# javieryu/nn_distributed_training

Hardware: NVIDIA H100
Metric: consensus node-rounds/sec (DiNNO, dist_mnist_PAPER; rounds/sec x graph nodes) (higher is better)
Workload: dtype fp64

## Files before the change

### nn_distributed_training_b200/ops/csrc/mnist_cl64.cu

```cuda
#include "mnist_device.cuh"

namespace nndt {
namespace mnist {

namespace cl64 {

constexpr int NT = 512, CL = 4, CELLS = 36, KC = 108, WS = 116, HS = 68;
constexpr int PXR = 10 * HW;
constexpr int KT = (KC + 7) / 8;
constexpr int HR = 68;
NNDT_DEVINL int hr(int j) { return (j >> 4) * 17 + (j & 15); }
constexpr int PART_WC = 0, PART_BC = 75, PART_B1 = 78, PART_W2 = 142, PART_B2 = 782, PART_LOSS = 792, PART_N = 793;

template <int MS>
struct Smem {
  static constexpr int NO = MS / CL;
  static constexpr bool kDoublePix = MS <= 32;
  static constexpr int PXS = kDoublePix ? PXR + 2 : PXR;
  double w[HID * WS];
  double a[MS * WS];
  double h[MS * HS];
  alignas(16) unsigned char img[kDoublePix ? MS * PXS * 8 : MS * PXS];
  double lut[kDoublePix ? 1 : 256];
  double h_loc[NO * HR > CL * 80 ? NO * HR : CL * 80];
  double dh_loc[NO * HID];
  double part[800];
  double w2[NCLS * HR];
  alignas(16) double b1[HID];
  alignas(16) double b2[16];
  double wc[80];
  double dz[NO * 16];
  double red[NO];
  int sidx[MS];
  int label[MS];
  float valid[MS];
  unsigned char arg[MS * KC];
};
static_assert(sizeof(Smem<16>) <= 227 * 1024 && sizeof(Smem<32>) <= 227 * 1024 && sizeof(Smem<64>) <= 227 * 1024,
              "shared memory budget");

NNDT_DEVINL double wmax(double v) {
#pragma unroll
  for (int o = 16; o > 0; o >>= 1) v = fmax(v, __shfl_xor_sync(0xffffffffu, v, o));
  return v;
}
template <int H>
NNDT_DEVINL void fold_half(double (&v)[16], int lane) {
  const bool up = (lane & (2 * H)) != 0;
#pragma unroll
  for (int i = 0; i < H; ++i) {
    const double send = up ? v[i] : v[i + H], keep = up ? v[i + H] : v[i];
    v[i] = keep + __shfl_xor_sync(0xffffffffu, send, 2 * H);
  }
}
NNDT_DEVINL void warp_reduce_scatter16(double (&v)[16], int lane) {
  fold_half<8>(v, lane); fold_half<4>(v, lane); fold_half<2>(v, lane); fold_half<1>(v, lane);
  v[0] += __shfl_xor_sync(0xffffffffu, v[0], 1);
}
NNDT_DEVINL void stamp(long long* prof, int idx, int tid) {
  if (prof != nullptr && tid == 0) {
    long long t;
    asm volatile("mov.u64 %0, %%globaltimer;" : "=l"(t));
    prof[idx] = t;
  }
}

template <int MS>
__global__ void __cluster_dims__(CL, 1, 1) __launch_bounds__(NT, 1)
mnist_cl64_train_kernel(const Args a, const GenericShape gs) {
  using SM = Smem<MS>;
  constexpr int NO = SM::NO, PXS = SM::PXS;
  constexpr bool kDoublePix = SM::kDoublePix;
  static_assert(MS % 16 == 0 && NO <= NT / 32, "tile geometry");
  static_assert(CELLS % 2 == 0 && NCLS % 2 == 0 && 32 + NCLS / 2 <= NT, "16-byte parameter copies");
  extern __shared__ __align__(16) unsigned char smem_raw[];
  SM& sm = *reinterpret_cast<SM*>(smem_raw);
  const int tid = threadIdx.x, warp = tid >> 5, lane = tid & 31;
  const int l = blockIdx.z, bsplit = blockIdx.y, nsplit = gridDim.y;
  const int c = (int)cluster_rank();
  const double* th = reinterpret_cast<const double*>(a.theta) + (size_t)l * a.n_pad;
  const double pmean = gs.mean, pis = gs.inv_std;
  const bool u8 = a.x_is_u8 != 0;
  double* imgd = reinterpret_cast<double*>(sm.img);
  auto pix = [&](int s, int p) -> double {
    if constexpr (kDoublePix) return imgd[s * PXS + p];
    else if (u8) return sm.lut[sm.img[s * PXR + p]];
    else return (double)__ldg(reinterpret_cast<const float*>(a.x) + (size_t)sm.sidx[s] * 784 + 6 * HW * c + p);
  };
  long long* prof = a.prof != nullptr ? a.prof + ((l * nsplit + bsplit) * CL + c) * 64 : nullptr;
  stamp(prof, 0, tid);

  const int call = a.calls != nullptr ? a.calls[l] : 0;
  const BatchGeom bg = batch_geom<true>(a, l, call);
  if (tid < MS) {
    int idx = 0, lab = 0; float ok = 0.f;
    const uint32_t t = (uint32_t)(bsplit * MS + tid);
    if (t < bg.bs) {
      ok = 1.f;
      idx = a.direct ? (int)(l * a.batch + t) : bg.shard_off + (int)feistel_permute(bg.start + t, bg.m, bg.key);
      lab = (int)a.y[idx];
    }
    sm.sidx[tid] = idx; sm.valid[tid] = ok; sm.label[tid] = lab;
  }
  if constexpr (!kDoublePix)
    if (tid < 256) sm.lut[tid] = ((double)tid * (1.0 / 255.0) - pmean) * pis;
  __syncthreads();
  constexpr int NU8 = (MS * 35 + NT - 1) / NT, NF4 = kDoublePix ? (MS * 70 + NT - 1) / NT : 1;
  uint2 pu[NU8]; float4 pf[NF4];
  if (u8) {
#pragma unroll
    for (int i = 0; i < NU8; ++i) {
      const int o = tid + i * NT;
      pu[i] = make_uint2(0, 0);
      if (o < MS * 35) {
        const int s = o / 35, q = o - s * 35;
        if (sm.valid[s] != 0.f)
          pu[i] = *reinterpret_cast<const uint2*>(reinterpret_cast<const unsigned char*>(a.x) + (size_t)sm.sidx[s] * 784 + 6 * HW * c + 8 * q);
      }
    }
  } else if constexpr (kDoublePix) {
#pragma unroll
    for (int i = 0; i < NF4; ++i) {
      const int o = tid + i * NT;
      pf[i] = make_float4(0.f, 0.f, 0.f, 0.f);
      if (o < MS * 70) {
        const int s = o / 70, q = o - s * 70;
        if (sm.valid[s] != 0.f)
          pf[i] = *reinterpret_cast<const float4*>(reinterpret_cast<const float*>(a.x) + (size_t)sm.sidx[s] * 784 + 6 * HW * c + 4 * q);
      }
    }
  }
  if (u8) {
#pragma unroll
    for (int i = 0; i < NU8; ++i) {
      const int o = tid + i * NT;
      if (o < MS * 35) {
        const int s = o / 35, q = o - s * 35;
        if constexpr (kDoublePix) {
          const uint32_t w[2] = {pu[i].x, pu[i].y};
          double* dst = imgd + s * PXS + 8 * q;
#pragma unroll
          for (int j = 0; j < 8; ++j) dst[j] = ((double)((w[j >> 2] >> (8 * (j & 3))) & 0xff) * (1.0 / 255.0) - pmean) * pis;
        } else {
          *reinterpret_cast<uint2*>(sm.img + s * PXR + 8 * q) = pu[i];
        }
      }
    }
  } else if constexpr (kDoublePix) {
#pragma unroll
    for (int i = 0; i < NF4; ++i) {
      const int o = tid + i * NT;
      if (o < MS * 70) {
        double* dst = imgd + (o / 70) * PXS + 4 * (o % 70);
        dst[0] = pf[i].x; dst[1] = pf[i].y; dst[2] = pf[i].z; dst[3] = pf[i].w;
      }
    }
  }
  stamp(prof, 1, tid);
  pdl_wait();
  pdl_launch_dependents();
  stamp(prof, 2, tid);

  constexpr int NW2 = (NCLS * HID + NT - 1) / NT;
  double wcv = 0.0, w2v[NW2];
  if (tid < 75) wcv = __ldcg(th + a.off_wc + tid);
  else if (tid < 78) wcv = __ldcg(th + a.off_bc + (tid - 75));
#pragma unroll
  for (int i = 0; i < NW2; ++i) {
    const int o = tid + i * NT;
    w2v[i] = o < NCLS * HID ? __ldcg(th + a.off_w2 + o) : 0.0;
  }
  for (int o = tid; o < HID * KC / 2; o += NT) {
    const int j = o / (KC / 2), r = o - j * (KC / 2), ch = r / (CELLS / 2), q = 2 * (r - ch * (CELLS / 2));
    cp_async16(sm.w + j * WS + ch * CELLS + q, th + a.off_w1 + (size_t)j * FC1_IN + ch * NPOOL + CELLS * c + q);
  }
  if (tid < HID / 2) cp_async16(sm.b1 + 2 * tid, th + a.off_b1 + 2 * tid);
  else if (tid >= 32 && tid < 32 + NCLS / 2) cp_async16(sm.b2 + 2 * (tid - 32), th + a.off_b2 + 2 * (tid - 32));
  cp_async_commit();
  if (tid < 78) sm.wc[tid] = wcv;
#pragma unroll
  for (int i = 0; i < NW2; ++i) {
    const int o = tid + i * NT;
    if (o < NCLS * HID) sm.w2[(o / HID) * HR + hr(o % HID)] = w2v[i];
  }
  __syncthreads();
  stamp(prof, 3, tid);

  for (int it = tid; it < MS * CELLS; it += NT) {
    const int s = it / CELLS, cell = it - s * CELLS;
    const int pr = cell / PHW, px = cell - pr * PHW;
    const int p0 = (2 * pr) * HW + 2 * px;
    double patch[6][6];
    if constexpr (kDoublePix) {
      const double* src = imgd + s * PXS + p0;
#pragma unroll
      for (int r = 0; r < 6; ++r)
#pragma unroll
        for (int q = 0; q < 6; q += 2) {
          const double2 v = *reinterpret_cast<const double2*>(src + r * HW + q);
          patch[r][q] = v.x; patch[r][q + 1] = v.y;
        }
    } else {
#pragma unroll
      for (int r = 0; r < 6; ++r)
#pragma unroll
        for (int q = 0; q < 6; ++q) patch[r][q] = pix(s, p0 + r * HW + q);
    }
    const bool ok = sm.valid[s] != 0.f;
#pragma unroll 1
    for (int ch = 0; ch < F; ++ch) {
      double a00 = 0, a01 = 0, a10 = 0, a11 = 0;
#pragma unroll
      for (int ky = 0; ky < KS; ++ky)
#pragma unroll
        for (int kx = 0; kx < KS; ++kx) {
          const double w = sm.wc[ch * 25 + ky * 5 + kx];
          a00 += w * patch[ky][kx]; a01 += w * patch[ky][kx + 1];
          a10 += w * patch[ky + 1][kx]; a11 += w * patch[ky + 1][kx + 1];
        }
      double m = a00; int ai = 0;
      if (a01 > m) { m = a01; ai = 1; }
      if (a10 > m) { m = a10; ai = 2; }
      if (a11 > m) { m = a11; ai = 3; }
      m += sm.wc[75 + ch];
      m = (ok && m > 0.0) ? m : 0.0;
      sm.a[s * WS + ch * CELLS + cell] = m;
      sm.arg[s * KC + ch * CELLS + cell] = (unsigned char)(ai | (m > 0.0 ? 4 : 0));
    }
  }
  cp_async_wait<0>();
  __syncthreads();
  stamp(prof, 4, tid);

  {
    constexpr int NJ1 = MS == 64 ? 2 : 1, NGRP = 8 / NJ1;
    if (warp < (MS / 16) * NGRP) {
      const int m0 = 16 * (warp / NGRP), n0 = 8 * NJ1 * (warp % NGRP);
      double acc[NJ1][4];
      zero(acc);
      gemm<NJ1>(acc, m0, n0, KC, lane, at(sm.a, WS), at_t(sm.w, WS));
#pragma unroll
      for (int j = 0; j < NJ1; ++j)
#pragma unroll
        for (int i = 0; i < 4; ++i) sm.h[frow(m0, lane, i) * HS + fcol(n0 + 8 * j, lane, i)] = acc[j][i];
    }
  }
  stamp(prof, 5, tid);
  cluster_sync();
  stamp(prof, 6, tid);
  if (c == 0 && tid == 0 && a.calls != nullptr) {
    if (a.arrive == nullptr || nsplit == 1) a.calls[l] = call + 1;
    else if (atomicAdd(a.arrive + l, 1u) == (unsigned)nsplit - 1) { a.arrive[l] = 0; a.calls[l] = call + 1; }
  }

  const int s0 = c * NO;
  const double inv_bs = 1.0 / (double)(bg.bs ? bg.bs : 1);
  if (warp < NO) {
    const int sl = warp, s = s0 + sl;
    double hv[2];
#pragma unroll
    for (int q = 0; q < 2; ++q) {
      const int j = lane + 32 * q;
      const double* src = sm.h + s * HS + j;
      double v = sm.b1[j];
#pragma unroll
      for (int r = 0; r < CL; ++r) v += ld_dsmem(map_to(src, (uint32_t)r));
      hv[q] = v > 0.0 ? v : 0.0;
      sm.h_loc[sl * HR + hr(j)] = hv[q];
    }
    __syncwarp();
    double zp[2];
#pragma unroll
    for (int r = 0; r < 2; ++r) {
      const int o = lane + 32 * r, cc = o >> 2, part = o & 3;
      double v = 0.0;
      if (o < 4 * NCLS) {
#pragma unroll
        for (int jj = 0; jj < 16; ++jj) v += sm.h_loc[sl * HR + part * 17 + jj] * sm.w2[cc * HR + part * 17 + jj];
      }
      v += __shfl_xor_sync(0xffffffffu, v, 1);
      v += __shfl_xor_sync(0xffffffffu, v, 2);
      zp[r] = v;
    }
    static_assert(NCLS > 8 && NCLS <= 16, "two rounds of four lanes per class");
    const double z0 = __shfl_sync(0xffffffffu, zp[0], (4 * lane) & 31), z1 = __shfl_sync(0xffffffffu, zp[1], (4 * lane) & 31);
    const bool cls = lane < NCLS;
    const double zc = cls ? (lane < 8 ? z0 : z1) + sm.b2[lane] : -1.0e300;
    const double mx = wmax(zc);
    const double se = warp_sum(cls ? exp(zc - mx) : 0.0);
    const double lse = mx + log(se);
    const int y = sm.label[s];
    const double ok = (double)sm.valid[s];
    const double dzc = cls ? ok * inv_bs * (exp(zc - lse) - (lane == y ? 1.0 : 0.0)) : 0.0;
    if (cls) sm.dz[sl * 16 + lane] = dzc;
    if (lane == y) sm.red[sl] = ok * (lse - zc);
    double dh[2] = {0.0, 0.0};
#pragma unroll
    for (int cc = 0; cc < NCLS; ++cc) {
      const double d = __shfl_sync(0xffffffffu, dzc, cc);
      dh[0] += d * sm.w2[cc * HR + hr(lane)];
      dh[1] += d * sm.w2[cc * HR + hr(lane + 32)];
    }
#pragma unroll
    for (int q = 0; q < 2; ++q) sm.dh_loc[sl * HID + lane + 32 * q] = hv[q] > 0.0 ? dh[q] : 0.0;
  }
  __syncthreads();
  for (int o = tid; o < NCLS * HID; o += NT) {
    const int cc = o >> 6, j = o & 63;
    double v = 0.0;
    for (int sl = 0; sl < NO; ++sl) v += sm.dz[sl * 16 + cc] * sm.h_loc[sl * HR + hr(j)];
    sm.part[PART_W2 + o] = v;
  }
  if (tid < HID) {
    double v = 0.0;
    for (int sl = 0; sl < NO; ++sl) v += sm.dh_loc[sl * HID + tid];
    sm.part[PART_B1 + tid] = v;
  } else if (tid >= 64 && tid < 64 + NCLS) {
    double v = 0.0;
    for (int sl = 0; sl < NO; ++sl) v += sm.dz[sl * 16 + (tid - 64)];
    sm.part[PART_B2 + (tid - 64)] = v;
  } else if (tid == 96) {
    double v = 0.0;
    for (int sl = 0; sl < NO; ++sl) v += sm.red[sl];
    sm.part[PART_LOSS] = v * inv_bs;
  }
  stamp(prof, 7, tid);
  cluster_sync();
  stamp(prof, 8, tid);
  double* gp = reinterpret_cast<double*>(a.grad_part) + ((size_t)l * nsplit + bsplit) * a.n_pad;
  {
    constexpr int NE = PART_N - PART_B1, PER = (NE + CL - 1) / CL;
    const int o = PART_B1 + c * PER + tid;
    if (tid < PER && o < PART_N) {
      double v = 0.0;
#pragma unroll
      for (int r = 0; r < CL; ++r) v += ld_dsmem(map_to(sm.part + o, (uint32_t)r));
      if (o < PART_W2) gp[a.off_b1 + (o - PART_B1)] = v;
      else if (o < PART_B2) gp[a.off_w2 + (o - PART_W2)] = v;
      else if (o < PART_LOSS) gp[a.off_b2 + (o - PART_B2)] = v;
      else {
        a.loss_part[l * nsplit + bsplit] = (float)v;
        if (a.loss_mirror != nullptr) a.loss_mirror[l * nsplit + bsplit] = (float)v;
      }
    }
  }
  for (int o = tid; o < MS * HID; o += NT) {
    const int s = o >> 6, j = o & 63, r = s / NO;
    sm.h[s * HS + j] = ld_dsmem(map_to(sm.dh_loc + (s - r * NO) * HID + j, (uint32_t)r));
  }
  __syncthreads();
  stamp(prof, 9, tid);

  constexpr int NP2 = (MS / 16) * (KT / 2), NR2 = (NP2 + NT / 32 - 1) / (NT / 32);
  static_assert(KT % 2 == 0 && KC * MS + (NT / 32) * 16 <= HID * WS, "da1 and the conv-grad warp sums fit in the W slice");
  double acc2[NR2][2][4];
#pragma unroll
  for (int r = 0; r < NR2; ++r) {
    zero(acc2[r]);
    const int p = warp + r * (NT / 32);
    if (p < NP2) gemm<2>(acc2[r], 16 * (p / (KT / 2)), 16 * (p % (KT / 2)), HID, lane, at(sm.h, HS), at(sm.w, WS));
  }
  __syncthreads();
  stamp(prof, 10, tid);
  double* da1 = sm.w;
#pragma unroll
  for (int r = 0; r < NR2; ++r) {
    const int p = warp + r * (NT / 32);
    if (p < NP2) {
      const int m0 = 16 * (p / (KT / 2)), n0 = 16 * (p % (KT / 2));
#pragma unroll
      for (int jt = 0; jt < 2; ++jt)
#pragma unroll
        for (int i = 0; i < 4; ++i) {
          const int s = frow(m0, lane, i), k = fcol(n0 + 8 * jt, lane, i);
          if (k < KC) da1[k * MS + s] = (sm.arg[s * KC + k] & 4) ? acc2[r][jt][i] : 0.0;
        }
    }
  }
  __syncthreads();
  stamp(prof, 11, tid);
  {
    constexpr int NP3 = (HID / 16) * (KT / 2);
#pragma unroll 1
    for (int p = warp; p < NP3; p += NT / 32) {
      const int m0 = 16 * (p / (KT / 2)), n0 = 16 * (p % (KT / 2));
      double acc[2][4];
      zero(acc);
      gemm<2>(acc, m0, n0, MS, lane, at_t(sm.h, HS), at(sm.a, WS));
#pragma unroll
      for (int jt = 0; jt < 2; ++jt)
#pragma unroll
        for (int i = 0; i < 4; i += 2) {
          const int j = frow(m0, lane, i), k = fcol(n0 + 8 * jt, lane, i);
          if (k < KC) {
            const int ch = k / CELLS, cell = k - ch * CELLS;
            *reinterpret_cast<double2*>(gp + a.off_w1 + (size_t)j * FC1_IN + ch * NPOOL + CELLS * c + cell) =
                make_double2(acc[jt][i], acc[jt][i + 1]);
          }
        }
    }
  }
  constexpr int KW = 3, NRUN = MS * 3;
  static_assert(KS * KW < NT / 32 && F * KS <= 16, "conv-grad work split");
  double* wsums = sm.w + KC * MS;
  auto pix2 = [&](int s, int p) -> double2 {
    if constexpr (kDoublePix) return *reinterpret_cast<const double2*>(imgd + s * PXS + p);
    else return make_double2(pix(s, p), pix(s, p + 1));
  };
  if (warp < KS * KW) {
    const int ky = warp / KW;
    double acc[16];
#pragma unroll
    for (int i = 0; i < 16; ++i) acc[i] = 0.0;
#pragma unroll 1
    for (int r = tid - ky * KW * 32; r < NRUN; r += KW * 32) {
      const int s = r % MS, pr = r / MS;
      const int rb = (2 * pr + ky) * HW;
      double x0[6], x1[6];
#pragma unroll
      for (int px = 0; px < PHW; ++px) {
        const int p = rb + 2 * px;
        if (px == 0) {
#pragma unroll
          for (int q = 0; q < 6; q += 2) {
            const double2 u = pix2(s, p + q), v = pix2(s, p + HW + q);
            x0[q] = u.x; x0[q + 1] = u.y; x1[q] = v.x; x1[q + 1] = v.y;
          }
        } else {
#pragma unroll
          for (int q = 0; q < 4; ++q) { x0[q] = x0[q + 2]; x1[q] = x1[q + 2]; }
          const double2 u = pix2(s, p + 4), v = pix2(s, p + HW + 4);
          x0[4] = u.x; x0[5] = u.y; x1[4] = v.x; x1[5] = v.y;
        }
#pragma unroll
        for (int ch = 0; ch < F; ++ch) {
          const int k = ch * CELLS + pr * PHW + px;
          const double g = da1[k * MS + s];
          const int ai = sm.arg[s * KC + k] & 3;
          const double g00 = ai == 0 ? g : 0.0, g01 = ai == 1 ? g : 0.0, g10 = ai == 2 ? g : 0.0, g11 = ai == 3 ? g : 0.0;
#pragma unroll
          for (int kx = 0; kx < KS; ++kx) {
            double& t = acc[ch * KS + kx];
            t = fma(g00, x0[kx], t); t = fma(g01, x0[kx + 1], t);
            t = fma(g10, x1[kx], t); t = fma(g11, x1[kx + 1], t);
          }
        }
      }
    }
    warp_reduce_scatter16(acc, lane);
    if ((lane & 1) == 0 && (lane >> 1) < F * KS) wsums[warp * 16 + (lane >> 1)] = acc[0];
  } else if (warp == KS * KW) {
#pragma unroll 1
    for (int ch = 0; ch < F; ++ch) {
      double v = 0.0;
      for (int o = lane; o < CELLS * MS; o += 32) v += da1[ch * CELLS * MS + o];
      v = warp_sum(v);
      if (lane == 0) wsums[warp * 16 + ch] = v;
    }
  }
  __syncthreads();
  if (tid < 78) {
    double v = 0.0;
    if (tid < 75) {
      const int ch = tid / 25, t = tid - ch * 25, ky = t / KS, kx = t - ky * KS;
#pragma unroll
      for (int w = 0; w < KW; ++w) v += wsums[(ky * KW + w) * 16 + ch * KS + kx];
    } else {
      v = wsums[KS * KW * 16 + (tid - 75)];
    }
    st_dsmem(map_to(sm.h_loc + c * 80 + tid, 0u), v);
  }
  stamp(prof, 12, tid);
  cluster_sync();
  if (c == 0 && tid < 78) {
    double v = 0.0;
#pragma unroll
    for (int r = 0; r < CL; ++r) v += sm.h_loc[r * 80 + tid];
    gp[tid < 75 ? a.off_wc + tid : a.off_bc + (tid - 75)] = v;
  }
  stamp(prof, 13, tid);
}

template <int MS>
static cudaError_t prepare_ms() {
  static cudaError_t prep = cudaFuncSetAttribute(mnist_cl64_train_kernel<MS>, cudaFuncAttributeMaxDynamicSharedMemorySize, (int)sizeof(Smem<MS>));
  return prep;
}

template <int MS>
static cudaError_t launch_ms(const Args& a, const GenericShape& gs, cudaStream_t st) {
  const cudaError_t prep = prepare_ms<MS>();
  if (prep != cudaSuccess) return prep;
  cudaLaunchConfig_t cfg{};
  cfg.gridDim = dim3(CL, 64 / MS, a.L); cfg.blockDim = dim3(NT);
  cfg.dynamicSmemBytes = sizeof(Smem<MS>); cfg.stream = st;
  cudaLaunchAttribute attr[1];
  attr[0].id = cudaLaunchAttributeProgrammaticStreamSerialization;
  attr[0].val.programmaticStreamSerializationAllowed = 1;
  static const bool no_pdl = getenv("NNDT_NO_PDL") != nullptr;
  cfg.attrs = attr; cfg.numAttrs = no_pdl ? 0 : 1;
  return cudaLaunchKernelEx(&cfg, mnist_cl64_train_kernel<MS>, a, gs);
}

template <int MS>
static int max_clusters_ms() {
  if (prepare_ms<MS>() != cudaSuccess) { cudaGetLastError(); return 0; }
  cudaLaunchConfig_t cfg{};
  cfg.gridDim = dim3(CL, 1, 1); cfg.blockDim = dim3(NT); cfg.dynamicSmemBytes = sizeof(Smem<MS>);
  int n = 0;
  if (cudaOccupancyMaxActiveClusters(&n, mnist_cl64_train_kernel<MS>, &cfg) != cudaSuccess) { cudaGetLastError(); return 0; }
  return n;
}

}

cudaError_t launch_train_cl64(const Args& a, const GenericShape& gs, int nsplit, cudaStream_t st) {
  switch (nsplit) {
    case 1: return cl64::launch_ms<64>(a, gs, st);
    case 2: return cl64::launch_ms<32>(a, gs, st);
    case 4: return cl64::launch_ms<16>(a, gs, st);
  }
  return cudaErrorInvalidValue;
}

int cl64_max_active_clusters(int nsplit) {
  switch (nsplit) {
    case 1: return cl64::max_clusters_ms<64>();
    case 2: return cl64::max_clusters_ms<32>();
    case 4: return cl64::max_clusters_ms<16>();
  }
  return 0;
}

int cl64_cluster_ctas() { return cl64::CL; }

}
}
```

Measured before the change: 151,200.

## Add compile-time-K register-prefetched DMMA gemm and overlap dW1 with conv grad

Adds a gemm_k helper with a compile-time K that prefetches the next k-step's A/B fragments into registers before issuing the f64 mma, and uses it for the forward FC1, backward dA and dW1 GEMMs. The dW1 GEMM is moved onto the last HID/16 warps, each owning a full row block across all N, so it can run concurrently with the conv-grad warps at the low warp indices instead of being striped across all warps first. The dW1 global stores switch to __stcg (cache-global) and profiling stamp indices shift. This is meant to hide shared-memory load latency and overlap the two backward phases, at the cost of more registers per warp and fewer warps on the dW1 GEMM.

```diff
diff --git a/nn_distributed_training_b200/ops/csrc/mnist_cl64.cu b/nn_distributed_training_b200/ops/csrc/mnist_cl64.cu
--- a/nn_distributed_training_b200/ops/csrc/mnist_cl64.cu
+++ b/nn_distributed_training_b200/ops/csrc/mnist_cl64.cu
@@ -57,6 +57,36 @@
   fold_half<8>(v, lane); fold_half<4>(v, lane); fold_half<2>(v, lane); fold_half<1>(v, lane);
   v[0] += __shfl_xor_sync(0xffffffffu, v[0], 1);
 }
+NNDT_DEVINL void dmma_nv(double (&c)[4], double a0, double a1, double b) {
+  asm("mma.sync.aligned.m16n8k4.row.col.f64.f64.f64.f64 {%0,%1,%2,%3}, {%4,%5}, {%6}, {%0,%1,%2,%3};"
+      : "+d"(c[0]), "+d"(c[1]), "+d"(c[2]), "+d"(c[3])
+      : "d"(a0), "d"(a1), "d"(b));
+}
+template <int NJ, int K, class FA, class FB>
+NNDT_DEVINL void gemm_k(double (&c)[NJ][4], int m0, int n0, int lane, FA A, FB B) {
+  static_assert(K % 4 == 0, "k steps of 4");
+  const int g = lane >> 2, t = lane & 3;
+  double a0 = A(m0 + g, t), a1 = A(m0 + g + 8, t), b[NJ];
+#pragma unroll
+  for (int j = 0; j < NJ; ++j) b[j] = B(t, n0 + 8 * j + g);
+#pragma unroll
+  for (int k0 = 0; k0 < K; k0 += 4) {
+    double na0 = 0.0, na1 = 0.0, nb[NJ];
+    if (k0 + 4 < K) {
+      const int k = k0 + 4 + t;
+      na0 = A(m0 + g, k); na1 = A(m0 + g + 8, k);
+#pragma unroll
+      for (int j = 0; j < NJ; ++j) nb[j] = B(k, n0 + 8 * j + g);
+    }
+#pragma unroll
+    for (int j = 0; j < NJ; ++j) dmma_nv(c[j], a0, a1, b[j]);
+    if (k0 + 4 < K) {
+      a0 = na0; a1 = na1;
+#pragma unroll
+      for (int j = 0; j < NJ; ++j) b[j] = nb[j];
+    }
+  }
+}
 NNDT_DEVINL void stamp(long long* prof, int idx, int tid) {
   if (prof != nullptr && tid == 0) {
     long long t;
@@ -238,7 +268,7 @@
       const int m0 = 16 * (warp / NGRP), n0 = 8 * NJ1 * (warp % NGRP);
       double acc[NJ1][4];
       zero(acc);
-      gemm<NJ1>(acc, m0, n0, KC, lane, at(sm.a, WS), at_t(sm.w, WS));
+      gemm_k<NJ1, KC>(acc, m0, n0, lane, at(sm.a, WS), at_t(sm.w, WS));
 #pragma unroll
       for (int j = 0; j < NJ1; ++j)
 #pragma unroll
@@ -358,7 +388,7 @@
   for (int r = 0; r < NR2; ++r) {
     zero(acc2[r]);
     const int p = warp + r * (NT / 32);
-    if (p < NP2) gemm<2>(acc2[r], 16 * (p / (KT / 2)), 16 * (p % (KT / 2)), HID, lane, at(sm.h, HS), at(sm.w, WS));
+    if (p < NP2) gemm_k<2, HID>(acc2[r], 16 * (p / (KT / 2)), 16 * (p % (KT / 2)), lane, at(sm.h, HS), at(sm.w, WS));
   }
   __syncthreads();
   stamp(prof, 10, tid);
@@ -379,26 +409,27 @@
   }
   __syncthreads();
   stamp(prof, 11, tid);
-  {
-    constexpr int NP3 = (HID / 16) * (KT / 2);
+  constexpr int W3 = NT / 32 - HID / 16, NJ3 = KT / 2;
+  if (warp >= W3) {
+    const int m0 = 16 * (warp - W3);
 #pragma unroll 1
-    for (int p = warp; p < NP3; p += NT / 32) {
-      const int m0 = 16 * (p / (KT / 2)), n0 = 16 * (p % (KT / 2));
-      double acc[2][4];
+    for (int n0 = 0; n0 < 8 * KT; n0 += 8 * NJ3) {
+      double acc[NJ3][4];
       zero(acc);
-      gemm<2>(acc, m0, n0, MS, lane, at_t(sm.h, HS), at(sm.a, WS));
-#pragma unroll
-      for (int jt = 0; jt < 2; ++jt)
+      gemm_k<NJ3, MS>(acc, m0, n0, lane, at_t(sm.h, HS), at(sm.a, WS));
+#pragma unroll
+      for (int jt = 0; jt < NJ3; ++jt)
 #pragma unroll
         for (int i = 0; i < 4; i += 2) {
           const int j = frow(m0, lane, i), k = fcol(n0 + 8 * jt, lane, i);
           if (k < KC) {
             const int ch = k / CELLS, cell = k - ch * CELLS;
-            *reinterpret_cast<double2*>(gp + a.off_w1 + (size_t)j * FC1_IN + ch * NPOOL + CELLS * c + cell) =
-                make_double2(acc[jt][i], acc[jt][i + 1]);
+            __stcg(reinterpret_cast<double2*>(gp + a.off_w1 + (size_t)j * FC1_IN + ch * NPOOL + CELLS * c + cell),
+                   make_double2(acc[jt][i], acc[jt][i + 1]));
           }
         }
     }
+    stamp(prof, 12, tid - W3 * 32);
   }
   constexpr int KW = 3, NRUN = MS * 3;
   static_assert(KS * KW < NT / 32 && F * KS <= 16, "conv-grad work split");
@@ -470,7 +501,7 @@
     }
     st_dsmem(map_to(sm.h_loc + c * 80 + tid, 0u), v);
   }
-  stamp(prof, 12, tid);
+  stamp(prof, 13, tid);
   cluster_sync();
   if (c == 0 && tid < 78) {
     double v = 0.0;
@@ -478,7 +509,7 @@
     for (int r = 0; r < CL; ++r) v += sm.h_loc[r * 80 + tid];
     gp[tid < 75 ? a.off_wc + tid : a.off_bc + (tid - 75)] = v;
   }
-  stamp(prof, 13, tid);
+  stamp(prof, 14, tid);
 }
 
 template <int MS>
```

After: 161,300 (median of 6 runs). 1.07x the previous value.
